# digitalcytometry/cytospace

Measured on AMD Instinct MI355X. Metric: cell-to-spot assignments/sec on NxN synthetic cost; bit-exact vs lapjv, higher is better.
Workload: dtype f32

## Files before the change

### cytospace_amd/_lib.py

```python
import ctypes
import os

_HERE = os.path.dirname(os.path.abspath(__file__))
LIB_PATH = os.environ.get("CYTOHIP_LIB") or os.path.join(_HERE, "libcytohip.so")
_lib = None

CYTO_OK = 0
CYTO_ERR_NONFINITE = 2
_EXC = {1: ValueError, 2: ValueError, 3: MemoryError, 7: ValueError, 8: ValueError}
CYTO_ERR_PEER = 9
CYTO_ERR_UNSUPPORTED = 7
CYTO_DTYPE_F32, CYTO_DTYPE_F64, CYTO_DTYPE_U16, CYTO_DTYPE_U8, CYTO_DTYPE_I32, CYTO_DTYPE_I64 = range(6)
CYTO_MTX_ERR_FRACTION, CYTO_MTX_ERR_NONFINITE, CYTO_MTX_ERR_MAGNITUDE, CYTO_MTX_ERR_SQUARE, CYTO_MTX_ERR_IO = range(2, 7)
CYTO_CSV_ERR_FRACTION, CYTO_CSV_ERR_NONFINITE, CYTO_CSV_ERR_MAGNITUDE, CYTO_CSV_ERR_IO = 2, 3, 4, 6
CYTO_TEXT_FRACTIONS = 1


class CytoHipError(RuntimeError):
    pass


class LapInfo(ctypes.Structure):
    _fields_ = [("ms_colred", ctypes.c_double), ("ms_cache", ctypes.c_double), ("ms_chain", ctypes.c_double),
                ("ms_total", ctypes.c_double)] + \
# ... 86 lines not shown
        L.cyto_memcpy_d2h.argtypes = [vp, vp, ctypes.c_size_t, i32]
        L.cyto_device_synchronize.argtypes = [i32]
        for name in ("cyto_lap_f32", "cyto_lap_f64"):
            getattr(L, name).argtypes = [i32, vp, i64, i32, vp, vp, vp, vp, ctypes.POINTER(ctypes.c_double),
                                         ctypes.POINTER(LapInfo), i32, vp]
        for name in ("cyto_lap_f32_opts", "cyto_lap_f64_opts"):
            getattr(L, name).argtypes = [i32, vp, i64, i32, vp, vp, vp, vp, ctypes.POINTER(ctypes.c_double),
                                         ctypes.POINTER(LapInfo), i32, vp, ctypes.POINTER(LapOpts)]
            getattr(L, name).restype = ctypes.c_int
        L.cyto_lap_f32_rowmap.argtypes = [i32, vp, i64, i32, i32, vp, vp, vp, vp, vp, ctypes.POINTER(ctypes.c_double),
                                          ctypes.POINTER(LapInfo), i32, vp, ctypes.POINTER(LapOpts)]
        L.cyto_lap_f32_rowmap.restype = ctypes.c_int
        if hasattr(L, "cyto_wide_embedded_solves"):
            L.cyto_wide_embedded_solves.argtypes = []
            L.cyto_wide_embedded_solves.restype = ctypes.c_longlong
        for name in ("cyto_fused_cache_solves", "cyto_fused_cache_fallback_rows"):
            if hasattr(L, name):
                getattr(L, name).argtypes = []
                getattr(L, name).restype = ctypes.c_longlong
        L.cyto_trim_device_cache.argtypes = [i32]
        L.cyto_trim_device_cache.restype = ctypes.c_int
        if hasattr(L, "cyto_cache_poison"):
            L.cyto_cache_poison.argtypes = [i32]
            L.cyto_cache_poison.restype = ctypes.c_int
            for name in ("cyto_cache_poison_fills", "cyto_cache_poison_bytes"):
                getattr(L, name).argtypes = []
                getattr(L, name).restype = ctypes.c_longlong
            L.cyto_cache_peek.argtypes = [ctypes.c_size_t, vp, i32]
            L.cyto_cache_peek.restype = ctypes.c_int
        dp = ctypes.POINTER(ctypes.c_double)
        L.cyto_lap_f32_from_f64.argtypes = [i32, vp, i64, vp, vp, vp, vp, ctypes.POINTER(ctypes.c_double),
# ... 111 lines not shown
    raise _EXC.get(status, CytoHipError)(f"cytohip status {status}: {msg}")


def fused_cache_solves():
    return int(lib().cyto_fused_cache_solves())


def fused_cache_fallback_rows():
    return int(lib().cyto_fused_cache_fallback_rows())


def wide_embedded_solves():
    return int(lib().cyto_wide_embedded_solves())


def cache_poison(byte):
    check(lib().cyto_cache_poison(-1 if byte is None else int(byte)))


def cache_poison_fills():
    return int(lib().cyto_cache_poison_fills())


def cache_poison_bytes():
    return int(lib().cyto_cache_poison_bytes())


def cache_peek(nbytes, device_id=0):
    import numpy as np
    out = np.empty(int(nbytes), np.uint8)
# ... 119 lines not shown
```

### cytospace_amd/csrc/lap_dev.h

```cpp
#pragma once
#include "cyto_common.h"
#include <math.h>
#include <stddef.h>

namespace cyto {

enum { C_RT = 0, C_ARR, C_AUG_INIT, C_AUG_RELAX, C_AUGS, C_HOPS, C_FREE_CR, C_FREE_A1, C_FREE_A2, C_ROWS_READ, C_NCOUNTERS,
       C2_DENSE_REFRESH = C_NCOUNTERS, C2_AUG_SKIPPED, C2_NCOUNTERS,
       C2_AUG_DENSE = C2_NCOUNTERS, C2_AUG_SPARSE_INIT, C3_NCOUNTERS };
enum { WC_ROUNDS = 0, WC_BIDS, WC_RETIRED, WC_ACTIVE_LEFT, WC_FREE_ARR, WC_DENSE_ARR, WC_DENSE_AUG, WC_AUG_ROUNDS, WC_AUG_PROCESSED,
       WC_TRIVIAL, WC_VERIFY_PASSES, WC_AUG_LAUNCHES, WC_N };
enum { WT_LIST_ROUNDS = 0, WT_LIST_TICKS, WT_CHAIN_ROUNDS, WT_CHAIN_TICKS,
       WT_DEALS, WT_ARR_SETUP_TICKS, WT_ARR_TAIL_TICKS,
       WT_PAR_DISCARDED,
       WT_AUG_ROUNDS_TICKS, WT_AUG_VERIFY_TICKS, WT_AUG_FINISH_TICKS, WT_AUG_TRIVIAL_TICKS,
       WT_ARR_LAUNCHES, WT_SCALED, WT_PHASES,
       WT_PAR_BATCHES,
       WT_N };

struct LapStatus {
    int nonfinite;
    int status;
    double total;
    long long counters[C3_NCOUNTERS];
    int numfree;
    int wide_done;
    int lazy_done;
    int wide_embedded;
    int ngroups;
    int pad1_[3];
    long long wide[WC_N];
    long long timers[WT_N];
    unsigned char arr[128];
};
static_assert(sizeof(LapStatus) == 512, "LapStatus layout");
static_assert(offsetof(LapStatus, nonfinite) == 0 && offsetof(LapStatus, status) == 4 && offsetof(LapStatus, total) == 8, "LapStatus layout");
static_assert(offsetof(LapStatus, counters) == 16 && offsetof(LapStatus, numfree) == 128, "LapStatus layout");
static_assert(offsetof(LapStatus, wide_done) == 132 && offsetof(LapStatus, lazy_done) == 136, "LapStatus layout");
static_assert(offsetof(LapStatus, ngroups) == 144 && offsetof(LapStatus, wide) == 160, "LapStatus layout");
static_assert(offsetof(LapStatus, timers) == 256 && offsetof(LapStatus, arr) == 384, "LapStatus layout");
static_assert(C3_NCOUNTERS * 8 + 16 <= offsetof(LapStatus, numfree), "a new counter would overwrite numfree");
static_assert(WC_N * 8 + 160 <= offsetof(LapStatus, timers), "a new wide counter would overwrite the timers");
static_assert(WT_N == 16 && WT_N * 8 + 256 <= offsetof(LapStatus, arr), "a new timer would overwrite wide_arr's state");
__host__ __device__ __forceinline__ LapStatus *lap_status(char *misc) { return reinterpret_cast<LapStatus *>(misc); }

// ... 89 lines not shown
```

### cytospace_amd/csrc/lap_wide.hip

```cpp
#include "lap_dev.h"
#include "lap_wide.h"
#include <algorithm>
#include <atomic>
#include <chrono>
#include <mutex>
#include <thread>
#include <vector>

namespace cyto {

#define WIDE_FIELDS(P, S)                                                                                                  \
    S(int, n) S(int64_t, ld) P(const float, cost) P(const int32_t, rowmap) P(float, v) P(float, u) P(float, cassign)          \
    P(unsigned long long, label) P(unsigned long long, bid) P(int32_t, rowsol) P(int32_t, colsol) P(int32_t, matches)          \
    P(int32_t, freerows) P(int32_t, act0) P(int32_t, act1) P(int32_t, touched) P(int32_t, slot_j) P(float, slot_p)            \
    P(float, slot_c) P(uint32_t, cache_col) P(float, cache_val) P(char, misc) S(long long, max_rounds)                     \
    P(const int32_t, same_prev) P(int32_t, seg_sync) S(int, aug_seg) S(int, aug_waste) S(int, arr_waste) S(int, seg_quorum)   \
    P(char, sc) S(int, par_groups) P(char, par) P(char, scx) P(float, cache_red) P(const int32_t, inv_off) P(const unsigned long long, inv_ent)    \
    P(const int32_t, emb_longest)
#define WIDE_F_PTR(T, name) T *name;
#define WIDE_F_VAL(T, name) T name;
struct WideArgs { WIDE_FIELDS(WIDE_F_PTR, WIDE_F_VAL) };

constexpr size_t WIDE_SC_BYTES = 2048;

namespace {

constexpr int WT = 1024;
constexpr int WNW = WT / 64;
constexpr int RTB = 256;

template <typename T> __device__ __forceinline__ T ld_sc1(const T *p) { return __hip_atomic_load(p, __ATOMIC_RELAXED, __HIP_MEMORY_SCOPE_AGENT); }
template <typename T> __device__ __forceinline__ void st_sc1(T *p, T x) { __hip_atomic_store(p, x, __ATOMIC_RELAXED, __HIP_MEMORY_SCOPE_AGENT); }
__device__ __forceinline__ int64_t wrow_off(const int32_t *__restrict__ rowmap, int i, int64_t ld) {
// ... 1010 lines not shown

size_t wide_aug_lds_bytes(int n, bool vlds, bool clds) {
    const size_t nblk = ((size_t)n + 63) / 64, nw32 = ((size_t)n + 31) / 32, npad = ((size_t)n + 3) & ~(size_t)3;
    return ((nblk * 8 + 3 * nw32 * 4 + npad * ((vlds ? 4 : 0) + (clds ? 2 : 0)) + 15) / 16) * 16;
}
bool wide_aug_vlds(int n) { return n <= 65534 && wide_aug_lds_bytes(n, true, true) + 4096 <= (size_t)LDS_DYNAMIC_MAX; }
bool wide_aug_clds(int n) { return n <= 65534 && wide_aug_lds_bytes(n, false, true) + 4096 <= (size_t)LDS_DYNAMIC_MAX; }

struct AugShared {
    unsigned long long T;
    int ntouch, any[3], npk[3], fail, anydense, rootdense, doroot, f, err;
    int waste, stop;
    int nhop;
    int nset;
    int scans;
    int st_row[64], st_col[64];
    float st_val[64];
};
static_assert(WNW * AP <= 32, "the queue of a round's full-row relaxations: two halves of the 64-entry staging arrays");

struct ParCtl {
    unsigned int bar_arrive, bar_gen;
    int P[2], nplog[2], nolog[2];
    int err, pad_;
    long long c_relax, c_hops, c_proc, c_dense, c_rounds, c_verify, c_batches, c_discarded;
};
static_assert(sizeof(ParCtl) <= 256, "control block");
constexpr int PAR_GMAX = 64;
#ifdef CYTO_AUG_FIN_SPLIT
constexpr int FS_MAXB = 2048, FS_G = 16, FS_NP = 14;
enum { FS_CLAIM, FS_WAIT1, FS_CHECK, FS_WAIT2, FS_UPDATE, FS_WALK, FS_COST, FS_RESET, FS_WAIT3, FS_REPAIR, FS_NTOUCH, FS_SETTLED, FS_HOPS, FS_ARRIVE };
__device__ long long g_fs[FS_MAXB][FS_G][FS_NP];
#define FS_OK (PAR && batchno - 1 < FS_MAXB && g < FS_G)
#define FS_BEGIN() { if (PAR && tid == 0) { fs_mark = wall_clock64(); if (FS_OK) g_fs[batchno - 1][g][FS_ARRIVE] = fs_mark; } }
#define FS_LAP(part) { if (PAR) { __syncthreads(); if (tid == 0) { const long long fsn_ = wall_clock64(); if (FS_OK) g_fs[batchno - 1][g][part] = fsn_ - fs_mark; fs_mark = fsn_; } } }
#define FS_SET(part, val) { if (tid == 0 && FS_OK) g_fs[batchno - 1][g][part] = (val); }
#define FS_COUNT() atomicAdd(&s.st_col[63], 1)
#else
#define FS_BEGIN()
#define FS_LAP(part)
#define FS_SET(part, val)
#define FS_COUNT()
#endif
static size_t wide_par_state_bytes(int n, int G) {
    const size_t np = ((size_t)n + 63) & ~(size_t)63;
    return 256 + (size_t)G * np * 8 + (size_t)G * np * 4 + (size_t)G * np * 8 + np * 4 + np * 8 + np * 8 + (size_t)G * np * 8 + (size_t)G * np * 8 +
// ... 108 lines not shown
typedef __attribute__((address_space(3))) unsigned long long lds_u64_t;
#ifndef CYTO_WALK_LINKS
#define CYTO_WALK_LINKS 1
#endif
#ifndef CYTO_WALK_HOP4
#define CYTO_WALK_HOP4 1
#endif
template <bool VLDS, bool CLDS, bool PAR>
__device__ __noinline__ unsigned long long search_end(const WideArgs *__restrict__ batch, lds_aug_t *sp, lds_u64_t *smem, int g_, int fr_, int batchno_,
                                                      unsigned pgen_, int active_) {
    constexpr bool LINKS = PAR && CYTO_WALK_LINKS;
    AugShared &s = *(AugShared *)sp;
    const int g = uni(g_), fr = uni(fr_), batchno = uni(batchno_);
    unsigned pgen = uni(pgen_);
    const bool active = uni(active_) != 0;
    const WideArgs a = load_wide_args(batch, PAR ? 0 : blockIdx.x);
    const int n = a.n, tid = threadIdx.x, lane = tid & 63, w = uni((int)(threadIdx.x >> 6));
    const int nblk = (n + 63) / 64, nw32 = (n + 31) / 32;
    const int G = PAR ? a.par_groups : 1;
    ParCtl *pc = reinterpret_cast<ParCtl *>(a.par);
    const SearchView sv(a, PAR, g);
    unsigned long long *lbl = sv.lbl, *setl = sv.setl, *link = sv.link;
    int32_t *tch = sv.tch, *hop_i = sv.hop_i, *hop_j = sv.hop_j;
    unsigned long long *bmin = (unsigned long long *)smem;
    uint32_t *dirty = reinterpret_cast<uint32_t *>(bmin + nblk);
    uint32_t *asg = dirty + nw32;
    uint32_t *dense = asg + nw32;
    float *s_v = reinterpret_cast<float *>(dense + nw32);
    uint16_t *s_cs = reinterpret_cast<uint16_t *>(s_v + (VLDS ? ((n + 3) & ~3) : 0));
    auto getv = [&](int j) -> float { return VLDS ? s_v[j] : ld_sc1(a.v + j); };
    auto is_asg = [&](int c) -> bool { return (asg[c >> 5] >> (c & 31)) & 1u; };
#ifdef CYTO_AUG_FIN_SPLIT
    long long fs_mark = 0;
#endif
    const unsigned long long Tk = active ? uni((unsigned long long)s.T) : ~0ull;
    const uint32_t Dord = (uint32_t)(Tk >> 32);
    const float D = ord2f(Dord);
    const int sink = (int)lid_of(Tk);
    const int nt = active ? uni(s.ntouch) : 0;
    const int par = batchno & 1;
    bool commit = true;
    int Pb = G;
    FS_BEGIN()
    if (PAR) {
        const bool have = Tk != ~0ull;
        if (active && !have && tid == 0) { atomicExch(&pc->err, 1); atomicMin(&pc->P[par], g); }
        const uint32_t key = ((uint32_t)batchno << 8) | (uint32_t)(255 - g);
        uint32_t fmin = PAR_GMAX + 1;
        auto flag = [&](uint32_t old) {
            if ((old >> 8) == (uint32_t)batchno && old != key) {
                const uint32_t go = 255u - (old & 255u);
                fmin = umin32(fmin, (uint32_t)g > go ? (uint32_t)g : go);
            }
        };
        if (have) {
            constexpr int CU_ = 4;
            for (int q0 = 0; q0 < nt; q0 += CU_ * WT) {
                int k[CU_], pre[CU_], cnt = 0;
                unsigned long long lb[CU_];
                uint64_t m[CU_];
                bool st[CU_];
// ... 184 lines not shown
        int k[4];
#pragma unroll
        for (int t = 0; t < 4; t++) { const int q = q0 + t * WT + tid; k[t] = q < nt ? ld_sc1(tch + q) : -1; }
#pragma unroll
        for (int t = 0; t < 4; t++)
            if (k[t] >= 0) {
                lbl[k[t]] = ~0ull;
                atomicAnd(&dirty[k[t] >> 5], ~(1u << (k[t] & 31)));
                bmin[k[t] >> 6] = ~0ull;
            }
    }
    if (s.anydense) for (int q = tid; q < nw32; q += WT) dense[q] = 0;
    __syncthreads();
    FS_SET(FS_NTOUCH, nt)
    FS_LAP(FS_RESET)
    return (unsigned long long)(uint32_t)nhop | ((unsigned long long)(uint32_t)Pb << 32) | ((unsigned long long)(commit ? 1 : 0) << 48);
}

constexpr int EMB_GATE = 4 * KCU;
template <bool VLDS, bool CLDS, bool PAR, bool EMB = false>
__global__ __launch_bounds__(WT) void wide_aug(const WideArgs *__restrict__ batch) {
    static_assert(!EMB || (PAR && !VLDS), "the embedded form: several searches at once, prices in global memory");
    extern __shared__ __align__(16) unsigned char w_smem[];
    __shared__ AugShared s;
    const int pstride = PAR ? (int)(gridDim.x / (unsigned)load_wide_args(batch, 0).par_groups) : 1;
    if (PAR && (blockIdx.x % pstride)) return;
    const int g = PAR ? uni((int)(blockIdx.x / pstride)) : 0;
    const WideArgs a = load_wide_args(batch, PAR ? 0 : blockIdx.x);
    if (PAR && a.emb_longest && (uni(ld_sc1(a.emb_longest)) <= EMB_GATE) != EMB) return;
    const int n = a.n, tid = threadIdx.x, lane = tid & 63, w = uni((int)(threadIdx.x >> 6));
    const int nblk = (n + 63) / 64, nw32 = (n + 31) / 32;
// ... 20 lines not shown
    }
    if (CLDS)
        for (int j = tid; j < n; j += WT) {
            if (VLDS) s_v[j] = a.v[j];
            const int o = a.colsol[j]; s_cs[j] = o < 0 ? (uint16_t)0xFFFFu : (uint16_t)o;
        }
    const int f0 = PAR ? 0 : lap_status(a.misc)->wide_done;
    if (!PAR) {
        long long *wc = lap_status(a.misc)->wide;
        if (wc[WC_AUG_LAUNCHES] > 0 && f0 >= numfree) {
            if (tid == 0 && a.seg_sync) a.seg_sync[1 + blockIdx.x] = 0;
            return;
        }
    }
    if (tid == 0) { s.waste = 0; s.stop = 0; }
    if (tid == 0) { s.T = ~0ull; s.ntouch = 0; s.any[0] = 0; s.any[1] = 0; s.any[2] = 0; s.npk[0] = 0; s.npk[1] = 0; s.npk[2] = 0; s.fail = 0; s.anydense = 0; s.rootdense = 0; s.doroot = 0; s.f = f0; s.err = 0; s.scans = 0; s.nset = 0; }
    __syncthreads();
    auto getv = [&](int j) -> float { return VLDS ? s_v[j] : ld_sc1(a.v + j); };
    auto getcs = [&](int j) -> int {
        if (CLDS) { const uint16_t x = s_cs[j]; return x == 0xFFFFu ? -1 : (int)x; }
        return ld_sc1(a.colsol + j);
    };
    auto is_asg = [&](int c) -> bool { return (asg[c >> 5] >> (c & 31)) & 1u; };

    long long c_relax = 0, c_hops = 0, c_rounds = 0, c_proc = 0, c_trivial = 0, c_dense = 0, c_verify = 0;
    long long t_rounds = 0, t_verify = 0, t_finish = 0, t_triv = 0, t_mark = wall_clock64();

#define AUG_LAP(acc) { const long long now_ = wall_clock64(); acc += now_ - t_mark; t_mark = now_; }
#ifdef CYTO_AUG_FIN_SPLIT
    long long fs_mark = 0;
    if (tid == 0) s.st_col[63] = 0;
// ... 14 lines not shown
            }
        }
    };
    auto relax_to = [&](int col, unsigned long long lv, int row) { after_offer(col, lv, row, offer(col, lv, row)); };

    int f = f0;
    int ph = 0;
    int rb[AP];
#pragma unroll
    for (int q = 0; q < AP; q++) rb[q] = -1;
    int seg_done = 0;
    int wact = 4;
    bool announced = false;
    int fbase = 0, batchno = 1, perr = 0;
    long long c_batches = 0, c_discarded = 0;
    for (;;) {
        if (!PAR && w == 0) {
            auto flush_one_edge = [&](int cnt) {
                if (lane < cnt) {
                    const int r = s.st_row[lane], cc = s.st_col[lane];
                    a.rowsol[r] = cc; a.colsol[cc] = r; a.cassign[cc] = s.st_val[lane];
                }
            };
            const int *remp = (a.same_prev && a.scx) ? cl_rem(a) : nullptr;
            int nst = 0;
            int p0, l0, r0, p1, l1, r1, p2, l2, r2, p3, l3v, r3v;
            uint32_t col0, col1, col2; float val0, val1, val2, vv0, vv1;
            auto start = [&](int ff) {
                auto len_of = [&](int pp) -> int { return pp < numfree ? (remp ? uni(remp[pp]) : 1) : 1; };
                auto row_at = [&](int pp) -> int { return pp < numfree ? uni(a.freerows[pp]) : -1; };
// ... 82 lines not shown
            } else if (lane < KCU && col != COLSENT) relax_to((int)col, (unsigned long long)f2ord(val - getv((int)col)) << 12, fr);
        }
        __syncthreads();

        for (;;) {
            int nd = 0;
            for (;;) {
                const unsigned long long Tlv = uni(lv_of(s.T));
                const int W = wact;
                if (w >= W && rb[0] < 0 && rb[1] < 0) {
                    __syncthreads();
                    const int any0 = uni(s.any[ph]), npd0 = uni(s.npk[ph]), np0 = npd0 & 0xFFFF;
                    ph = (ph + 1) % 3;
                    c_rounds++;
                    wact = np0 > 6 ? WNW : 4;
                    nd = npd0 >> 16;
                    if (!any0 || nd) break;
                    continue;
                }
                unsigned long long mk = ~0ull;
                if (w < W) for (int b = w + W * lane; b < nblk; b += W * 64) mk = umin64(mk, bmin[b]);
                bool pk[AP]; int pj[AP], oi[AP];
                unsigned long long lab[AP];
                float ca[AP], vp[AP], val[AP];
                uint32_t col[AP];
                {
                    uint32_t dk = lv_of(mk) < Tlv ? (uint32_t)(mk >> 32) : 0xFFFFFFFFu;
#pragma unroll
                    for (int q = 0; q < AP; q++) {
                        const uint32_t m = wave_min_u32(dk);
                        pk[q] = m != 0xFFFFFFFFu;
// ... 5 lines not shown
#pragma unroll
                for (int q = 0; q < AP; q++) {
                    if (pk[q] && lane == 0) { atomicAnd(&dirty[pj[q] >> 5], ~(1u << (pj[q] & 31))); bmin[pj[q] >> 6] = ~0ull; }
                }
                if (lane == 0 && (pk[0] || pk[1] || rb[0] >= 0 || rb[1] >= 0)) { s.any[ph] = 1; if (pk[0]) atomicAdd(&s.npk[ph], (int)pk[0] + (int)pk[1]); }
                asm volatile("s_waitcnt lgkmcnt(0)" ::: "memory");
                int pjx[AP];
                unsigned long long lab_r[AP];
                float ca_r[AP], vp_r[AP];
                int oi_r[AP];
#pragma unroll
                for (int q = 0; q < AP; q++) {
                    pjx[q] = pk[q] ? pj[q] : 0;
                    lab_r[q] = ld_sc1(lbl + pjx[q]); ca_r[q] = ld_sc1(a.cassign + pjx[q]);
                }
                bool db[AP]; unsigned long long lbr[AP];
#pragma unroll
                for (int q = 0; q < AP; q++) {
                    const int c = (rb[q] < 0 ? 0 : rb[q]) * 64 + lane;
                    db[q] = rb[q] >= 0 && c < n && ((dirty[c >> 5] >> (c & 31)) & 1u);
                    lbr[q] = ld_sc1(lbl + (db[q] ? c : pjx[q]));
                }
#pragma unroll
                for (int q = 0; q < AP; q++) { vp_r[q] = getv(pjx[q]); oi_r[q] = getcs(pjx[q]); }
#pragma unroll
                for (int q = 0; q < AP; q++) {
                    oi[q] = uni(oi_r[q]);
                    const int oix = oi[q] < 0 ? 0 : oi[q];
                    col[q] = a.cache_col[(int64_t)oix * KC + lane];
                    val[q] = EMB ? ld_sc1(a.cache_red + (int64_t)oix * KC + lane) : a.cache_val[(int64_t)oix * KC + lane];
                }
#pragma unroll
                for (int q = 0; q < AP; q++) {
                    lab[q] = pk[q] ? uni(lab_r[q]) : ~0ull; ca[q] = uni(ca_r[q]); vp[q] = uni(vp_r[q]);
                    if (!pk[q]) { col[q] = COLSENT; oi[q] = 0; }
                }
                unsigned long long old[AP], co[AP];
                bool off[AP], dn[AP];
                float vc[AP];
#pragma unroll
                for (int q = 0; q < AP; q++) {
                    const bool valid = lane < KCU && col[q] != COLSENT;
                    vc[q] = EMB ? 0.0f : getv(valid ? (int)col[q] : pjx[q]);
                }
#pragma unroll
                for (int q = 0; q < AP; q++) {
                    off[q] = false; dn[q] = false; old[q] = 0; co[q] = 0;
                    const uint32_t dord = (uint32_t)(lab[q] >> 32), kq = (uint32_t)(lab[q] >> 20) & LKMAX;
                    if (pk[q] && lv_of(lab[q]) < Tlv) {
                        c_proc++;
                        if ((dense[oi[q] >> 5] >> (oi[q] & 31)) & 1u) { dn[q] = true; continue; }
// ... 24 lines not shown
                        old[0] = off[0] ? r0 : 0; old[1] = off[1] ? r1 : 0;
                    }
                }
#pragma unroll
                for (int q = 0; q < AP; q++) {
                    const bool better = off[q] && (lkey(co[q], (uint32_t)oi[q]) < old[q]);
                    if (__ballot(better) && better) after_offer((int)col[q], co[q], oi[q], old[q]);
                }
#pragma unroll
                for (int q = 0; q < AP; q++) {
                    if (!dn[q]) continue;
                    const uint32_t dord = (uint32_t)(lab[q] >> 32), kq = (uint32_t)(lab[q] >> 20) & LKMAX;
                    const float h = (ca[q] - vp[q]) - ord2f(dord);
                    if (n >= COOP_MIN_N) {
                        if (lane == 0) {
                            const int e = atomicAdd(&s.npk[ph], 1 << 16) >> 16;
                            s.st_row[e] = oi[q]; s.st_row[32 + e] = pj[q]; s.st_col[e] = (int)dord; s.st_col[32 + e] = (int)kq; s.st_val[e] = h;
                        }
                    } else {
                        const float *__restrict__ row = a.cost + wrow_off(a.rowmap, oi[q], a.ld);
                        const int pjq = pj[q], oiq = oi[q];
                        wave_row_sweep(row, n, lane, [&](int c, float x) {
                            const unsigned long long lv = edge_lv(f2ord((x - getv(c)) - h), dord, kq);
                            if (c != pjq && lv <= lv_of(s.T) && (lkey(lv, (uint32_t)oiq) < ld_sc1(lbl + c))) relax_to(c, lv, oiq);
                        });
                    }
                    c_dense++;
                    if (lane == 0) atomicAdd(&s.waste, 1);
                }
#pragma unroll
                for (int q = 0; q < AP; q++) {
// ... 2 lines not shown
                        const uint32_t dk = db[q] ? (uint32_t)(lbr[q] >> 32) : 0xFFFFFFFFu;
                        const uint32_t m = wave_min_u32(dk);
                        if (m != 0xFFFFFFFFu) {
                            const int l = __ffsll((unsigned long long)__ballot(dk == m)) - 1;
                            if (lane == 0) atomicMin(&bmin[rb[q]], ((unsigned long long)m << 32) | (uint32_t)(c - lane + l));
                        }
                    }
                    rb[q] = pk[q] ? (pj[q] >> 6) : -1;
                }
                __syncthreads();
                const int any = uni(s.any[ph]), npd = uni(s.npk[ph]), np = npd & 0xFFFF;
                if (tid == 0) { s.any[(ph + 2) % 3] = 0; s.npk[(ph + 2) % 3] = 0; }
                ph = (ph + 1) % 3;
                c_rounds++;
                wact = np > 6 ? WNW : 4;
                nd = npd >> 16;
                if (!any || nd) break;
            }
            if (nd) {
                coop_dense_rows<VLDS>(&s, nd, a.cost, a.rowmap, a.ld, n, w, lane, lbl, tch, dirty, bmin, asg, s_v, a.v);
                continue;
            }
            AUG_LAP(t_rounds)
            const unsigned long long Tk = s.T;
            const uint32_t Dord = (uint32_t)(Tk >> 32);
            const float D = Tk == ~0ull ? INFINITY : ord2f(Dord);
            const int nt = s.ntouch;
            for (int q = tid; q < nt; q += WT) {
                const int k = ld_sc1(tch + q);
                const unsigned long long lbk = ld_sc1(lbl + k);
                const uint32_t dord = (uint32_t)(lbk >> 32);
                if (lv_of(lbk) < lv_of(Tk) && is_asg(k)) {
// ... 20 lines not shown
                    if (lv <= lv_of(s.T) && (lkey(lv, (uint32_t)fr) < ld_sc1(lbl + c))) relax_to(c, lv, fr);
                }
            __syncthreads();
            if (tid == 0) { if (fail) s.anydense = 1; s.fail = 0; s.doroot = 0; }
            __syncthreads();
            AUG_LAP(t_verify)
            if (!fail) break;
        }

        }

        const unsigned long long Tk = active ? s.T : ~0ull;
        if (!PAR && Tk == ~0ull) { if (tid == 0) s.err = 1; __syncthreads(); break; }
        const unsigned long long er = uni(search_end<VLDS, CLDS, PAR>(batch, (lds_aug_t *)&s, (lds_u64_t *)w_smem, g, fr, batchno, pgen, active ? 1 : 0));
        if (PAR) pgen++;
        const bool commit = (er >> 48) & 1;
        const int Pb = (int)((er >> 32) & 0xFFFFu);
        const int par = batchno & 1;
        c_hops += (long long)(uint32_t)er;
        if (PAR && active && !commit) c_discarded++;
        if (tid == 0) { if (commit) c_relax += s.scans; s.scans = 0; s.T = ~0ull; s.ntouch = 0; s.nset = 0; s.anydense = 0; s.rootdense = 0; s.f = f + 1; }
        f++;
        __syncthreads();
#ifdef CYTO_AUG_FIN_SPLIT
        if (PAR && tid == 0) fs_mark = wall_clock64();
#endif
        if (PAR) {
            par_barrier(pc, G, pgen);
            perr = uni(ld_sc1(&pc->err));
            const int npl = uni(ld_sc1(&pc->nplog[par])), nol = uni(ld_sc1(&pc->nolog[par]));
// ... 29 lines not shown

    __syncthreads();
    __shared__ double s_tot[WNW];
    __shared__ long long s_wc[WNW][4];
    if (lane == 0) { s_wc[w][0] = c_proc; s_wc[w][1] = c_dense; s_wc[w][2] = c_trivial; s_wc[w][3] = (w == 0) ? c_hops : 0; }
    __syncthreads();
    long long proc = 0, dn = 0, triv = 0, hops0 = 0;
    for (int k = 0; k < WNW; k++) { proc += s_wc[k][0]; dn += s_wc[k][1]; triv += s_wc[k][2]; hops0 += s_wc[k][3]; }
    if (PAR) {
        if (tid == 0) {
            atomicAdd(reinterpret_cast<unsigned long long *>(&pc->c_relax), (unsigned long long)c_relax);
            atomicAdd(reinterpret_cast<unsigned long long *>(&pc->c_hops), (unsigned long long)hops0);
            atomicAdd(reinterpret_cast<unsigned long long *>(&pc->c_proc), (unsigned long long)proc);
            atomicAdd(reinterpret_cast<unsigned long long *>(&pc->c_dense), (unsigned long long)dn);
            atomicAdd(reinterpret_cast<unsigned long long *>(&pc->c_discarded), (unsigned long long)c_discarded);
            if (g == 0) { pc->c_rounds = c_rounds; pc->c_verify = c_verify; pc->c_batches = c_batches; }
        }
        par_barrier(pc, G, pgen);
        if (g != 0) return;
        c_relax = (long long)ld_sc1(reinterpret_cast<unsigned long long *>(&pc->c_relax));
        hops0 = (long long)ld_sc1(reinterpret_cast<unsigned long long *>(&pc->c_hops));
        proc = (long long)ld_sc1(reinterpret_cast<unsigned long long *>(&pc->c_proc));
        dn = (long long)ld_sc1(reinterpret_cast<unsigned long long *>(&pc->c_dense));
        f = perr || ld_sc1(&pc->err) ? f : numfree;
    }
    double tot = 0.0;
    for (int i = tid; i < n; i += WT) {
        const int j = ld_sc1(a.rowsol + i);
        if (j >= 0) {
            const float cij = ld_sc1(a.cassign + j);
// ... 8 lines not shown
    if (tid == 0) {
        double t = 0.0;
        for (int k = 0; k < WNW; k++) t += s_tot[k];
        const bool err = s.err || (PAR && (perr || ld_sc1(&pc->err)));
        LapStatus *st = lap_status(a.misc);
        st->total = t;
        long long *ctr = st->counters, *wc = st->wide;
        ctr[C_AUG_INIT] = numfree; ctr[C_AUG_RELAX] += c_relax; ctr[C_AUGS] = numfree; ctr[C_HOPS] += hops0;
        wc[WC_DENSE_AUG] += dn; wc[WC_AUG_LAUNCHES] += 1; wc[WC_AUG_ROUNDS] += c_rounds; wc[WC_AUG_PROCESSED] += proc; wc[WC_TRIVIAL] += triv; wc[WC_VERIFY_PASSES] += c_verify;
        if (err) st->status = 1;
        st->wide_done = err ? numfree : f;
        if (a.seg_sync) a.seg_sync[1 + (PAR ? 0 : blockIdx.x)] = err ? 0 : numfree - f;
        long long *tmr = st->timers;
        tmr[WT_AUG_ROUNDS_TICKS] += t_rounds; tmr[WT_AUG_VERIFY_TICKS] += t_verify; tmr[WT_AUG_FINISH_TICKS] += t_finish; tmr[WT_AUG_TRIVIAL_TICKS] += t_triv;
        if (PAR) st->wide_embedded = EMB ? 1 : 0;
        if (PAR) { tmr[WT_PAR_BATCHES] = ld_sc1(reinterpret_cast<unsigned long long *>(&pc->c_batches)); tmr[WT_PAR_DISCARDED] = ld_sc1(reinterpret_cast<unsigned long long *>(&pc->c_discarded)); }
    }
}

__device__ __forceinline__ int nth_set(unsigned long long m, int k) {
    for (int t = 0; t < k && m; t++) m &= m - 1;
    return m ? __ffsll((long long)m) - 1 : -1;
}

__global__ __launch_bounds__(HEADB) void wide_claim_lists(const WideArgs *__restrict__ batch) {
    const WideArgs a = load_wide_args(batch, blockIdx.y);
    const int numfree = lap_status(a.misc)->numfree;
    const int lane = threadIdx.x & 63;
    const int gw = blockIdx.x * (HEADB / 64) + (threadIdx.x >> 6), nw = gridDim.x * (HEADB / 64);
    if (blockIdx.x == 0 && threadIdx.x == 0) { ClaimCtl *c = cl_ctl(a); c->changed = 0; c->blocked = 0x7FFFFFFF; c->rounds = 0; }
// ... 331 lines not shown
}
static int32_t *emb_counts(const WideArgs &wa, int n) { return reinterpret_cast<int32_t *>(reinterpret_cast<char *>(wa.cache_red) + emb_off_cnt(n)); }
static int wide_build_embedded(const WideArgs &wa, int n, hipStream_t stream) {
    char *eb = reinterpret_cast<char *>(wa.cache_red);
    int32_t *cnt = emb_counts(wa, n), *bsum = reinterpret_cast<int32_t *>(eb + emb_off_bsum(n)), *rank = reinterpret_cast<int32_t *>(eb + emb_off_rank(n));
    const int nb = emb_blocks(n);
    CYTO_HIP(hipMemsetAsync(cnt, 0, ((size_t)n + 1) * 4, stream));
    hipLaunchKernelGGL(embed_red_count, dim3((n + 3) / 4), dim3(256), 0, stream, n, wa.cache_col, wa.cache_val, wa.v, wa.cache_red, cnt, rank);
    hipLaunchKernelGGL(embed_block_sums, dim3(nb), dim3(EMB_SB), 0, stream, n, cnt, bsum);
    hipLaunchKernelGGL(embed_scan, dim3(nb), dim3(EMB_SB), 0, stream, n, cnt, bsum, const_cast<int32_t *>(wa.inv_off));
    hipLaunchKernelGGL(embed_fill, dim3((n + 3) / 4), dim3(256), 0, stream, n, wa.cache_col, wa.cache_val, wa.inv_off, rank, const_cast<unsigned long long *>(wa.inv_ent));
    CYTO_HIP(hipGetLastError());
    return CYTO_OK;
}
static std::atomic<long long> g_embedded_solves{0};

static void wide_aug_lds_choice(int n, bool &vlds, bool &clds) {
    const int lds_knob = CYTO_KNOB("CYTO_AUG_LDS").set ? CYTO_KNOB("CYTO_AUG_LDS").value : 2;
    vlds = lds_knob >= 2 && wide_aug_vlds(n); clds = lds_knob >= 1 && wide_aug_clds(n);
}

static int wide_launch_aug(const WideArgs *d_args, int nb, int n, hipStream_t stream, int par_groups, bool embed) {
    bool vlds, clds;
    wide_aug_lds_choice(n, vlds, clds);
    const size_t shm = wide_aug_lds_bytes(n, vlds, clds);
    if (shm > (size_t)LDS_DYNAMIC_MAX) return CYTO_ERR_UNSUPPORTED;
    if (par_groups > 1) {
        void (*k)(const WideArgs *) = vlds ? wide_aug<true, true, true> : clds ? wide_aug<false, true, true> : wide_aug<false, false, true>;
        if (embed) {
            if (vlds) return CYTO_ERR_INTERNAL;
// ... 83 lines not shown
        wa.cache_col = j.cache_col; wa.cache_val = j.cache_val; wa.misc = j.misc;
        wa.max_rounds = pl.rounds;
        wa.aug_seg = pl.rebuild;
        wa.aug_waste = (int)std::min<long long>(1 << 30, std::max<long long>(16, (2000000ll + (long long)nl * n * n / 100) / n));
        wa.arr_waste = std::max(8, wa.aug_waste / 3);
        if (CYTO_KNOB("CYTO_ARR_WASTE").set) wa.arr_waste = std::max(1, CYTO_KNOB("CYTO_ARR_WASTE").value);
        wa.seg_quorum = nl > 1 ? std::max(1, nl / 4) : 0;
        wa.seg_sync = nullptr;
        wa.same_prev = j.same;
        wa.sc = j.state->as<char>() + sc_off;
        CYTO_HIP(hipMemsetAsync(wa.sc, 0, WIDE_SC_BYTES, stream));
        wa.scx = j.state->as<char>() + scx_off;
        CYTO_HIP(hipMemsetAsync(wa.scx, 0, wide_sc_ext_bytes(n), stream));
        CYTO_HIP(hipMemsetAsync(wa.scx, 0xFF, wide_sc_ones_bytes(n), stream));
        wa.par_groups = parg; wa.par = nullptr;
        if (parg > 0) {
            const size_t np_ = ((size_t)n + 63) & ~(size_t)63;
            wa.par = j.state->as<char>() + par_off;
            CYTO_HIP(hipMemsetAsync(wa.par, 0, 256, stream));
            CYTO_HIP(hipMemsetD32Async(reinterpret_cast<hipDeviceptr_t>(wa.par + 8), WIDE_PAR_GMAX + 1, 2, stream));
            CYTO_HIP(hipMemsetAsync(wa.par + 256, 0xFF, (size_t)parg * np_ * 8, stream));
            CYTO_HIP(hipMemsetAsync(wa.par + 256 + (size_t)parg * np_ * 20, 0, np_ * 4, stream));
        }
        CYTO_HIP(hipMemcpyAsync(wa.cassign, wa.v, nT, hipMemcpyDeviceToDevice, stream));
        CYTO_HIP(hipMemsetAsync(wa.label, 0xFF, 2 * nT, stream));
        CYTO_HIP(hipMemsetAsync(wa.bid, 0xFF, 2 * nT, stream));
    }
    DevBuf d_wa, d_sync;
    if ((rc = d_wa.alloc(sizeof(WideArgs) * nl, stream)) || (rc = d_sync.alloc(sizeof(int32_t) * ((size_t)nl + 1), stream))) return rc;
    for (WideArgs &wa : h_wa) wa.seg_sync = d_sync.as<int32_t>();
// ... 34 lines not shown
            embed = true;
        }
        CYTO_HIP(hipMemsetAsync(d_sync.p, 0, sizeof(int32_t), stream));
        if ((rc = wide_launch_aug(d_wa.as<WideArgs>(), nl, n, stream, parg, embed))) return rc;
        if (embed && h_wa[0].emb_longest && (rc = wide_launch_aug(d_wa.as<WideArgs>(), nl, n, stream, parg, false))) return rc;
        if (parg > 0) { CYTO_HIP(hipStreamSynchronize(stream)); break; }
        CYTO_HIP(hipMemcpyAsync(h_sync.data(), d_sync.p, sizeof(int32_t) * ((size_t)nl + 1), hipMemcpyDeviceToHost, stream));
        CYTO_HIP(hipStreamSynchronize(stream));
        bool done = true;
        for (int k = 0; k < nl; k++) done = done && h_sync[(size_t)k + 1] == 0;
        if (done) break;
    }
    return CYTO_OK;
}

void wide_note_status(const LapStatus &h) { if (h.wide_embedded) g_embedded_solves.fetch_add(1); }

void wide_info(cyto_lap_info *info, const LapStatus &h) {
    const long long *wc = h.wide, *tm = h.timers;
    info->wide = 1;
    info->aug_handover = -1;
    info->wide_rounds = wc[WC_ROUNDS]; info->wide_retired = wc[WC_RETIRED]; info->wide_dense_arr = wc[WC_DENSE_ARR];
    info->wide_dense_aug = wc[WC_DENSE_AUG]; info->wide_aug_rounds = wc[WC_AUG_ROUNDS]; info->wide_aug_settled = wc[WC_AUG_PROCESSED];
    info->wide_trivial = wc[WC_TRIVIAL]; info->wide_verify_passes = wc[WC_VERIFY_PASSES]; info->wide_aug_launches = wc[WC_AUG_LAUNCHES];
    info->wide_list_rounds = tm[WT_LIST_ROUNDS]; info->wide_chain_rounds = tm[WT_CHAIN_ROUNDS];
    info->wide_ms_list = tm[WT_LIST_TICKS] * 1e-5; info->wide_ms_chain = tm[WT_CHAIN_TICKS] * 1e-5;
    info->wide_ms_aug_rounds = tm[WT_AUG_ROUNDS_TICKS] * 1e-5; info->wide_ms_aug_verify = tm[WT_AUG_VERIFY_TICKS] * 1e-5;
    info->wide_ms_aug_finish = tm[WT_AUG_FINISH_TICKS] * 1e-5; info->wide_ms_aug_trivial = tm[WT_AUG_TRIVIAL_TICKS] * 1e-5;
    info->wide_arr_launches = tm[WT_ARR_LAUNCHES]; info->wide_scaled = tm[WT_SCALED]; info->wide_phases = tm[WT_PHASES];
    info->wide_par_batches = tm[WT_PAR_BATCHES]; info->wide_par_discarded = tm[WT_PAR_DISCARDED];
}

}

extern "C" long long cyto_wide_embedded_solves(void) { return cyto::g_embedded_solves.load(); }

#ifdef CYTO_AUG_FIN_SPLIT
extern "C" int cyto_wide_fin_split(long long *out, int *max_batches, int *groups, int *parts) {
    using namespace cyto;
    *max_batches = FS_MAXB; *groups = FS_G; *parts = FS_NP;
    if (!out) return 0;
    if (hipDeviceSynchronize() != hipSuccess) return 5;
    if (hipMemcpyFromSymbol(out, HIP_SYMBOL(g_fs), sizeof(long long) * FS_MAXB * FS_G * FS_NP) != hipSuccess) return 5;
    void *p = nullptr;
    if (hipGetSymbolAddress(&p, HIP_SYMBOL(g_fs)) != hipSuccess || hipMemset(p, 0, sizeof(long long) * FS_MAXB * FS_G * FS_NP) != hipSuccess) return 5;
    return 0;
}
#endif
```

### include/cytohip.h

```cpp
#ifndef CYTOHIP_H
#define CYTOHIP_H

#include <stddef.h>
#include <stdint.h>

#ifdef __cplusplus
extern "C" {
#endif

enum {
    CYTO_OK = 0,
    CYTO_ERR_BAD_ARG = 1,
    CYTO_ERR_NONFINITE = 2,
    CYTO_ERR_NOMEM = 3,
    CYTO_ERR_INTERNAL = 4,
    CYTO_ERR_HIP = 5,
    CYTO_ERR_NO_DEVICE = 6,
    CYTO_ERR_UNSUPPORTED = 7,
    CYTO_ERR_SHAPE = 8,
    CYTO_ERR_PEER = 9
};

const char *cyto_strerror(int status);
const char *cyto_last_hip_error(void);
const char *cyto_version(void);
int cyto_abi_sizes(size_t *lap_info, size_t *lap_opts, size_t *assign_info, size_t *chunk);
long long cyto_wide_embedded_solves(void);
long long cyto_fused_cache_solves(void);
long long cyto_fused_cache_fallback_rows(void);

int cyto_device_count(int *count);
int cyto_device_name(int device_id, char *buf, size_t buflen);
int cyto_malloc(void **dptr, size_t bytes, int device_id);
int cyto_free(void *dptr, int device_id);
int cyto_memcpy_h2d(void *dst, const void *src, size_t bytes, int device_id);
int cyto_memcpy_d2h(void *dst, const void *src, size_t bytes, int device_id);
int cyto_memcpy_d2d(void *dst, const void *src, size_t bytes, int device_id);
int cyto_device_synchronize(int device_id);
int cyto_trim_device_cache(int device_id);
int cyto_cache_poison(int byte);
long long cyto_cache_poison_fills(void);
long long cyto_cache_poison_bytes(void);
// ... 307 lines not shown
```

Before: 1.366 million.

## Abort doomed speculative augmenting searches early in parallel wide solver

In the parallel batched augmentation, each group now checks the shared commit-prefix marker P during relaxation rounds. If a lower-indexed group has already failed, this group's result would be discarded, so it flags an abort bit and leaves its Dijkstra search early. The abort skips the error flag, resets the search state and counts aborted searches for diagnostics. The feature is on by default through a knob. This cuts wasted work on searches that will be thrown away, at the cost of an extra shared-memory load and atomic per round and added control complexity around correctness.

```diff
diff --git a/cytospace_amd/_lib.py b/cytospace_amd/_lib.py
--- a/cytospace_amd/_lib.py
+++ b/cytospace_amd/_lib.py
@@ -124,7 +124,7 @@
         if hasattr(L, "cyto_wide_embedded_solves"):
             L.cyto_wide_embedded_solves.argtypes = []
             L.cyto_wide_embedded_solves.restype = ctypes.c_longlong
-        for name in ("cyto_fused_cache_solves", "cyto_fused_cache_fallback_rows"):
+        for name in ("cyto_fused_cache_solves", "cyto_fused_cache_fallback_rows", "cyto_wide_aborted_searches"):
             if hasattr(L, name):
                 getattr(L, name).argtypes = []
                 getattr(L, name).restype = ctypes.c_longlong
@@ -266,6 +266,10 @@
     return int(lib().cyto_wide_embedded_solves())
 
 
+def wide_aborted_searches():
+    return int(lib().cyto_wide_aborted_searches())
+
+
 def cache_poison(byte):
     check(lib().cyto_cache_poison(-1 if byte is None else int(byte)))
 
diff --git a/cytospace_amd/csrc/lap_dev.h b/cytospace_amd/csrc/lap_dev.h
--- a/cytospace_amd/csrc/lap_dev.h
+++ b/cytospace_amd/csrc/lap_dev.h
@@ -28,7 +28,8 @@
     int lazy_done;
     int wide_embedded;
     int ngroups;
-    int pad1_[3];
+    int wide_aborted;
+    int pad1_[2];
     long long wide[WC_N];
     long long timers[WT_N];
     unsigned char arr[128];
diff --git a/cytospace_amd/csrc/lap_wide.hip b/cytospace_amd/csrc/lap_wide.hip
--- a/cytospace_amd/csrc/lap_wide.hip
+++ b/cytospace_amd/csrc/lap_wide.hip
@@ -16,7 +16,7 @@
     P(float, slot_c) P(uint32_t, cache_col) P(float, cache_val) P(char, misc) S(long long, max_rounds)                     \
     P(const int32_t, same_prev) P(int32_t, seg_sync) S(int, aug_seg) S(int, aug_waste) S(int, arr_waste) S(int, seg_quorum)   \
     P(char, sc) S(int, par_groups) P(char, par) P(char, scx) P(float, cache_red) P(const int32_t, inv_off) P(const unsigned long long, inv_ent)    \
-    P(const int32_t, emb_longest)
+    P(const int32_t, emb_longest) S(int, aug_abort)
 #define WIDE_F_PTR(T, name) T *name;
 #define WIDE_F_VAL(T, name) T name;
 struct WideArgs { WIDE_FIELDS(WIDE_F_PTR, WIDE_F_VAL) };
@@ -1057,6 +1057,7 @@
     int nhop;
     int nset;
     int scans;
+    int ab, nab;
     int st_row[64], st_col[64];
     float st_val[64];
 };
@@ -1066,13 +1067,14 @@
     unsigned int bar_arrive, bar_gen;
     int P[2], nplog[2], nolog[2];
     int err, pad_;
-    long long c_relax, c_hops, c_proc, c_dense, c_rounds, c_verify, c_batches, c_discarded;
+    long long c_relax, c_hops, c_proc, c_dense, c_rounds, c_verify, c_batches, c_discarded, c_aborted;
 };
 static_assert(sizeof(ParCtl) <= 256, "control block");
 constexpr int PAR_GMAX = 64;
 #ifdef CYTO_AUG_FIN_SPLIT
-constexpr int FS_MAXB = 2048, FS_G = 16, FS_NP = 14;
-enum { FS_CLAIM, FS_WAIT1, FS_CHECK, FS_WAIT2, FS_UPDATE, FS_WALK, FS_COST, FS_RESET, FS_WAIT3, FS_REPAIR, FS_NTOUCH, FS_SETTLED, FS_HOPS, FS_ARRIVE };
+constexpr int FS_MAXB = 2048, FS_G = 16, FS_NP = 15;
+enum { FS_CLAIM, FS_WAIT1, FS_CHECK, FS_WAIT2, FS_UPDATE, FS_WALK, FS_COST, FS_RESET, FS_WAIT3, FS_REPAIR, FS_NTOUCH, FS_SETTLED, FS_HOPS, FS_ARRIVE,
+       FS_ABORTED };
 __device__ long long g_fs[FS_MAXB][FS_G][FS_NP];
 #define FS_OK (PAR && batchno - 1 < FS_MAXB && g < FS_G)
 #define FS_BEGIN() { if (PAR && tid == 0) { fs_mark = wall_clock64(); if (FS_OK) g_fs[batchno - 1][g][FS_ARRIVE] = fs_mark; } }
@@ -1211,6 +1213,7 @@
     const int g = uni(g_), fr = uni(fr_), batchno = uni(batchno_);
     unsigned pgen = uni(pgen_);
     const bool active = uni(active_) != 0;
+    const bool aborted = PAR && active && uni(s.ab) != 0;
     const WideArgs a = load_wide_args(batch, PAR ? 0 : blockIdx.x);
     const int n = a.n, tid = threadIdx.x, lane = tid & 63, w = uni((int)(threadIdx.x >> 6));
     const int nblk = (n + 63) / 64, nw32 = (n + 31) / 32;
@@ -1230,7 +1233,7 @@
 #ifdef CYTO_AUG_FIN_SPLIT
     long long fs_mark = 0;
 #endif
-    const unsigned long long Tk = active ? uni((unsigned long long)s.T) : ~0ull;
+    const unsigned long long Tk = active && !aborted ? uni((unsigned long long)s.T) : ~0ull;
     const uint32_t Dord = (uint32_t)(Tk >> 32);
     const float D = ord2f(Dord);
     const int sink = (int)lid_of(Tk);
@@ -1241,7 +1244,8 @@
     FS_BEGIN()
     if (PAR) {
         const bool have = Tk != ~0ull;
-        if (active && !have && tid == 0) { atomicExch(&pc->err, 1); atomicMin(&pc->P[par], g); }
+        if (active && !have && tid == 0) { if (!aborted) atomicExch(&pc->err, 1); atomicMin(&pc->P[par], g); }
+        FS_SET(FS_ABORTED, aborted ? 1 : 0)
         const uint32_t key = ((uint32_t)batchno << 8) | (uint32_t)(255 - g);
         uint32_t fmin = PAR_GMAX + 1;
         auto flag = [&](uint32_t old) {
@@ -1456,7 +1460,8 @@
     __syncthreads();
     FS_SET(FS_NTOUCH, nt)
     FS_LAP(FS_RESET)
-    return (unsigned long long)(uint32_t)nhop | ((unsigned long long)(uint32_t)Pb << 32) | ((unsigned long long)(commit ? 1 : 0) << 48);
+    return (unsigned long long)(uint32_t)nhop | ((unsigned long long)(uint32_t)Pb << 32) | ((unsigned long long)(commit ? 1 : 0) << 48) |
+           ((unsigned long long)(aborted ? 1 : 0) << 49);
 }
 
 constexpr int EMB_GATE = 4 * KCU;
@@ -1507,7 +1512,7 @@
         }
     }
     if (tid == 0) { s.waste = 0; s.stop = 0; }
-    if (tid == 0) { s.T = ~0ull; s.ntouch = 0; s.any[0] = 0; s.any[1] = 0; s.any[2] = 0; s.npk[0] = 0; s.npk[1] = 0; s.npk[2] = 0; s.fail = 0; s.anydense = 0; s.rootdense = 0; s.doroot = 0; s.f = f0; s.err = 0; s.scans = 0; s.nset = 0; }
+    if (tid == 0) { s.T = ~0ull; s.ntouch = 0; s.any[0] = 0; s.any[1] = 0; s.any[2] = 0; s.npk[0] = 0; s.npk[1] = 0; s.npk[2] = 0; s.fail = 0; s.anydense = 0; s.rootdense = 0; s.doroot = 0; s.f = f0; s.err = 0; s.scans = 0; s.nset = 0; s.ab = 0; s.nab = 0; }
     __syncthreads();
     auto getv = [&](int j) -> float { return VLDS ? s_v[j] : ld_sc1(a.v + j); };
     auto getcs = [&](int j) -> int {
@@ -1552,6 +1557,8 @@
     bool announced = false;
     int fbase = 0, batchno = 1, perr = 0;
     long long c_batches = 0, c_discarded = 0;
+    constexpr int AUG_ABORT = 1 << 30;
+    const int gthr = PAR && a.aug_abort ? g : -1;
     for (;;) {
         if (!PAR && w == 0) {
             auto flush_one_edge = [&](int cnt) {
@@ -1664,7 +1671,7 @@
                     ph = (ph + 1) % 3;
                     c_rounds++;
                     wact = np0 > 6 ? WNW : 4;
-                    nd = npd0 >> 16;
+                    nd = PAR && (npd0 & AUG_ABORT) ? -1 : npd0 >> 16;
                     if (!any0 || nd) break;
                     continue;
                 }
@@ -1700,6 +1707,8 @@
                     pjx[q] = pk[q] ? pj[q] : 0;
                     lab_r[q] = ld_sc1(lbl + pjx[q]); ca_r[q] = ld_sc1(a.cassign + pjx[q]);
                 }
+                int p_r = PAR_GMAX + 1;
+                if (PAR && w == 0) p_r = ld_sc1(&pc->P[batchno & 1]);
                 bool db[AP]; unsigned long long lbr[AP];
 #pragma unroll
                 for (int q = 0; q < AP; q++) {
@@ -1721,6 +1730,7 @@
                     lab[q] = pk[q] ? uni(lab_r[q]) : ~0ull; ca[q] = uni(ca_r[q]); vp[q] = uni(vp_r[q]);
                     if (!pk[q]) { col[q] = COLSENT; oi[q] = 0; }
                 }
+                if (PAR && w == 0 && uni(p_r) <= gthr && lane == 0) atomicOr(&s.npk[ph], AUG_ABORT);
                 unsigned long long old[AP], co[AP];
                 bool off[AP], dn[AP];
                 float vc[AP];
@@ -1775,7 +1785,7 @@
                     const float h = (ca[q] - vp[q]) - ord2f(dord);
                     if (n >= COOP_MIN_N) {
                         if (lane == 0) {
-                            const int e = atomicAdd(&s.npk[ph], 1 << 16) >> 16;
+                            const int e = (atomicAdd(&s.npk[ph], 1 << 16) >> 16) & 0x3FFF;
                             s.st_row[e] = oi[q]; s.st_row[32 + e] = pj[q]; s.st_col[e] = (int)dord; s.st_col[32 + e] = (int)kq; s.st_val[e] = h;
                         }
                     } else {
@@ -1808,8 +1818,14 @@
                 ph = (ph + 1) % 3;
                 c_rounds++;
                 wact = np > 6 ? WNW : 4;
-                nd = npd >> 16;
+                nd = PAR && (npd & AUG_ABORT) ? -1 : npd >> 16;
                 if (!any || nd) break;
+            }
+            if (PAR && nd < 0) {
+                AUG_LAP(t_rounds)
+                if (tid == 0) s.ab = 1;
+                __syncthreads();
+                break;
             }
             if (nd) {
                 coop_dense_rows<VLDS>(&s, nd, a.cost, a.rowmap, a.ld, n, w, lane, lbl, tch, dirty, bmin, asg, s_v, a.v);
@@ -1860,6 +1876,12 @@
         if (!PAR && Tk == ~0ull) { if (tid == 0) s.err = 1; __syncthreads(); break; }
         const unsigned long long er = uni(search_end<VLDS, CLDS, PAR>(batch, (lds_aug_t *)&s, (lds_u64_t *)w_smem, g, fr, batchno, pgen, active ? 1 : 0));
         if (PAR) pgen++;
+        if (PAR && ((er >> 49) & 1)) {
+#pragma unroll
+            for (int q = 0; q < AP; q++) rb[q] = -1;
+            wact = 4;
+            if (tid == 0) { s.any[0] = 0; s.any[1] = 0; s.any[2] = 0; s.npk[0] = 0; s.npk[1] = 0; s.npk[2] = 0; s.ab = 0; s.nab++; }
+        }
         const bool commit = (er >> 48) & 1;
         const int Pb = (int)((er >> 32) & 0xFFFFu);
         const int par = batchno & 1;
@@ -1919,6 +1941,7 @@
             atomicAdd(reinterpret_cast<unsigned long long *>(&pc->c_proc), (unsigned long long)proc);
             atomicAdd(reinterpret_cast<unsigned long long *>(&pc->c_dense), (unsigned long long)dn);
             atomicAdd(reinterpret_cast<unsigned long long *>(&pc->c_discarded), (unsigned long long)c_discarded);
+            if (s.nab) atomicAdd(reinterpret_cast<unsigned long long *>(&pc->c_aborted), (unsigned long long)s.nab);
             if (g == 0) { pc->c_rounds = c_rounds; pc->c_verify = c_verify; pc->c_batches = c_batches; }
         }
         par_barrier(pc, G, pgen);
@@ -1957,6 +1980,7 @@
         long long *tmr = st->timers;
         tmr[WT_AUG_ROUNDS_TICKS] += t_rounds; tmr[WT_AUG_VERIFY_TICKS] += t_verify; tmr[WT_AUG_FINISH_TICKS] += t_finish; tmr[WT_AUG_TRIVIAL_TICKS] += t_triv;
         if (PAR) st->wide_embedded = EMB ? 1 : 0;
+        if (PAR) st->wide_aborted = (int)ld_sc1(reinterpret_cast<unsigned long long *>(&pc->c_aborted));
         if (PAR) { tmr[WT_PAR_BATCHES] = ld_sc1(reinterpret_cast<unsigned long long *>(&pc->c_batches)); tmr[WT_PAR_DISCARDED] = ld_sc1(reinterpret_cast<unsigned long long *>(&pc->c_discarded)); }
     }
 }
@@ -2318,6 +2342,7 @@
     return CYTO_OK;
 }
 static std::atomic<long long> g_embedded_solves{0};
+static std::atomic<long long> g_aborted_searches{0};
 
 static void wide_aug_lds_choice(int n, bool &vlds, bool &clds) {
     const int lds_knob = CYTO_KNOB("CYTO_AUG_LDS").set ? CYTO_KNOB("CYTO_AUG_LDS").value : 2;
@@ -2431,6 +2456,7 @@
         CYTO_HIP(hipMemsetAsync(wa.scx, 0, wide_sc_ext_bytes(n), stream));
         CYTO_HIP(hipMemsetAsync(wa.scx, 0xFF, wide_sc_ones_bytes(n), stream));
         wa.par_groups = parg; wa.par = nullptr;
+        wa.aug_abort = CYTO_KNOB("CYTO_AUG_ABORT").set ? (CYTO_KNOB("CYTO_AUG_ABORT").value != 0 ? 1 : 0) : 1;
         if (parg > 0) {
             const size_t np_ = ((size_t)n + 63) & ~(size_t)63;
             wa.par = j.state->as<char>() + par_off;
@@ -2495,7 +2521,10 @@
     return CYTO_OK;
 }
 
-void wide_note_status(const LapStatus &h) { if (h.wide_embedded) g_embedded_solves.fetch_add(1); }
+void wide_note_status(const LapStatus &h) {
+    if (h.wide_embedded) g_embedded_solves.fetch_add(1);
+    if (h.wide_aborted > 0) g_aborted_searches.fetch_add(h.wide_aborted);
+}
 
 void wide_info(cyto_lap_info *info, const LapStatus &h) {
     const long long *wc = h.wide, *tm = h.timers;
@@ -2515,6 +2544,7 @@
 }
 
 extern "C" long long cyto_wide_embedded_solves(void) { return cyto::g_embedded_solves.load(); }
+extern "C" long long cyto_wide_aborted_searches(void) { return cyto::g_aborted_searches.load(); }
 
 #ifdef CYTO_AUG_FIN_SPLIT
 extern "C" int cyto_wide_fin_split(long long *out, int *max_batches, int *groups, int *parts) {
diff --git a/include/cytohip.h b/include/cytohip.h
--- a/include/cytohip.h
+++ b/include/cytohip.h
@@ -26,6 +26,7 @@
 const char *cyto_version(void);
 int cyto_abi_sizes(size_t *lap_info, size_t *lap_opts, size_t *assign_info, size_t *chunk);
 long long cyto_wide_embedded_solves(void);
+long long cyto_wide_aborted_searches(void);
 long long cyto_fused_cache_solves(void);
 long long cyto_fused_cache_fallback_rows(void);
 
```

Result: faster. 1.401 million (median of 6 runs) (+2.6%).
